# HKUST-Aerial-Robotics/DenseSurfelMapping

Measured on AMD Instinct MI355X. Metric: depth frames fused/sec @ KITTI 1226x370, higher is better.
Workload: dtype f32

## Files before the change

densesurfelmapping_amd/csrc/dsm_api.hip:

```cpp
#include <hip/hip_runtime.h>

#include <cstdarg>
#include <cstdio>
#include <cstdlib>
#include <cstring>
#include <cstdint>
#include <new>
#include <algorithm>
#include <atomic>
#include <condition_variable>
#include <functional>
#include <mutex>
#include <string>
#include <thread>
#include <chrono>
#include <unordered_map>
#include <vector>

#include "dsm_components.h"
#include "dsm_device.h"
#include "dsm_frame_copy.h"
#include "dsm_frame_format.h"
#include "dsm_frame_rings.h"
#include "dsm_ranges.h"
// ... 1033 lines not shown
    CREATE_TRY(dev_alloc(h, &h->d_params, (size_t)kParamRing));
    c.params = h->d_params;
    h->ev_slot.assign((size_t)c.n_slots, nullptr);
    h->slot_used.assign((size_t)c.n_slots, 0);
    CREATE_TRY(hipEventCreateWithFlags(&h->ev_fence, hipEventDisableTiming));
    CREATE_TRY(dev_alloc(h, &h->d_stage_img, (size_t)w * hh));
    CREATE_TRY(dev_alloc(h, &h->d_stage_depth, (size_t)w * hh));
    int np = cfg->pipeline_depth > 0 ? cfg->pipeline_depth : 4;
    if (np != 1 && np != 2 && np != 4 && np != 8 && np != 12 && np != 16 && np != 24 && np != 32) { fail(h, DSM_E_INVALID, "pipeline_depth must be 1, 2, 4, 8, 12, 16, 24 or 32"); return bail(DSM_E_INVALID); }
    if ((cfg->flags & DSM_FLAG_WAVE_STAMPS) && !kWaveStamps) {
        fail(h, DSM_E_INVALID, "DSM_FLAG_WAVE_STAMPS: this library was built without phase stamps (-DDSM_WAVE_STAMPS=1: tools/wave_stamps.py builds such a copy)");
        return bail(DSM_E_INVALID);
    }
    h->n_pipe = np;
    if (np > 1) {
        CREATE_TRY(hipEventCreateWithFlags(&h->ev_params, hipEventDisableTiming));
        CREATE_TRY(hipStreamCreateWithFlags(&h->copy_stream, hipStreamNonBlocking));
    }
    for (int p = 0; p < np; p++) {
        dsm_handle::Pipe &pp = h->pipe[p];
        pp.ctx = c;
        DeviceCtx &q = pp.ctx;
        q.cursor_mul = np; q.cursor_add = p;
        if (np > 1) {
            if (np >= 4 && p < kBatchStreams - ((np == 12 || np == 24) ? 1 : 0)) pp.stream = batch_stream_at(h->device, p);
            if (pp.stream) pp.own_stream = false;
            else CREATE_TRY(hipStreamCreateWithFlags(&pp.stream, hipStreamNonBlocking));
            CREATE_TRY(hipEventCreateWithFlags(&pp.ev_sp, hipEventDisableTiming));
            CREATE_TRY(hipEventCreateWithFlags(&pp.ev_map, hipEventDisableTiming));
        }
        CREATE_TRY(dev_alloc(h, &q.label, (size_t)c.slot_elems));
        CREATE_TRY(dev_alloc(h, &q.cand, (size_t)c.slot_elems));
        CREATE_TRY(dev_alloc(h, &q.worklist, (size_t)c.slot_elems));
        CREATE_TRY(dev_alloc(h, &q.core, (size_t)c.n_seed));
        CREATE_TRY(dev_alloc(h, &q.inv_depth, (size_t)c.n_seed));
        CREATE_TRY(dev_alloc(h, &q.core_stage, (size_t)c.n_seed));
        CREATE_TRY(dev_alloc(h, &q.stable_stage, (size_t)c.n_seed));
        CREATE_TRY(dev_alloc(h, &q.tmin, (size_t)c.n_seed));
        CREATE_TRY(dev_alloc(h, &q.first_empty, (size_t)kSweeps * kWorkers));
        CREATE_TRY(dev_alloc(h, &q.gn_hdr, (size_t)c.n_seed));
        CREATE_TRY(dev_alloc(h, &q.normals, (size_t)c.slot_elems * 3));
        CREATE_TRY(dev_alloc(h, &q.plane, (size_t)c.n_seed));
        CREATE_TRY(dev_alloc(h, &q.seeds, (size_t)c.n_seed));
        CREATE_TRY(dev_alloc(h, &q.spawn_rec, (size_t)c.n_seed));
        CREATE_TRY(dev_alloc(h, &q.spawn_ok, (size_t)c.n_seed));
        CREATE_TRY(dev_alloc(h, &q.fused_flag, (size_t)c.n_seed));
        CREATE_TRY(dev_alloc(h, &q.seed_weight, (size_t)c.n_seed));
        CREATE_TRY(dev_alloc(h, &q.spawn_idx, (size_t)c.n_seed));
        int32_t *ps = nullptr;
        CREATE_TRY(dev_alloc(h, &ps, 64));
        q.work_count = ps + 0; q.cursor = ps + 8; q.fit_big_count = ps + 24; q.rest_count = ps + 32;
        q.fit_small_cap = kFitSmallCap;
        CREATE_TRY(dev_alloc(h, &q.cur, 1));
        CREATE_TRY(dev_alloc(h, &q.rest_list, (size_t)((c.n_seed + 63) / 64) * kRestListCap * 64));
        CREATE_TRY(dev_alloc(h, &q.inl_mask, (size_t)((c.n_seed + 63) / 64) * (2 * kCell) * 64));
        if ((cfg->flags & DSM_FLAG_WAVE_STAMPS) && kWaveStamps) CREATE_TRY(dev_alloc(h, &q.stamps, (size_t)5 * c.n_seed * 8));
        q.params = h->d_params;
        if (np > 1) CREATE_TRY(hipEventRecord(pp.ev_map, h->stream));
    }
    h->hc = h->pipe[0].ctx;
    if (np >= 4) {
        CREATE_TRY(dev_alloc(h, &h->d_pipe_ctxs, (size_t)np));
        DeviceCtx tmp[kMaxPipes];
        for (int p = 0; p < np; p++) tmp[p] = h->pipe[p].ctx;
        CREATE_TRY(hipMemcpyAsync(h->d_pipe_ctxs, tmp, sizeof(DeviceCtx) * (size_t)np, hipMemcpyHostToDevice, h->stream));
        CREATE_TRY(hipStreamSynchronize(h->stream));
    }
    CREATE_TRY(hipHostMalloc((void **)&h->h_params, sizeof(FrameParams) * kParamRing, hipHostMallocDefault));
    CREATE_TRY(hipHostMalloc((void **)&h->h_scalars, 512, hipHostMallocDefault));
    memset(h->h_scalars, 0, 512);
    for (int i = 0; i <= kNumStages + 1; i++) CREATE_TRY(hipEventCreate(&h->ev[i]));
    h->have_events = true;
    CREATE_TRY(hipStreamSynchronize(h->stream));
#undef CREATE_TRY
    (void)rc;
    {
        std::lock_guard<std::mutex> lk(g_live_mu);
        h->generation = g_next_generation++;
        g_live[h] = h->generation;
    }
    *out = h;
    return DSM_OK;
}

void dsm_destroy(dsm_handle *h) {
    if (!h) return;
    {
        std::lock_guard<std::mutex> lk(g_live_mu);
        g_live.erase(h);
    }
    (void)hipSetDevice(h->device);
    if (h->stream && h->batch_order_ev) (void)hipStreamWaitEvent(h->stream, h->batch_order_ev, 0);
    if (h->stream) (void)hipStreamSynchronize(h->stream);
    retire_graphs(h);
    for (int i = 0; i < 4; i++) {
        if (h->g_group[i]) (void)hipGraphExecDestroy(h->g_group[i]);
        if (h->g_group_map[i]) (void)hipGraphExecDestroy(h->g_group_map[i]);
        if (h->g_group_map_large[i]) (void)hipGraphExecDestroy(h->g_group_map_large[i]);
    }
    for (int p = 0; p < kMaxPipes; p++) {
        dsm_handle::Pipe &pp = h->pipe[p];
        if (pp.stream) (void)hipStreamSynchronize(pp.stream);
        if (pp.g_sp) (void)hipGraphExecDestroy(pp.g_sp);
        if (pp.g_sp_main) (void)hipGraphExecDestroy(pp.g_sp_main);
        for (int i = 0; i < 2; i++) {
            if (pp.g_map[i]) (void)hipGraphExecDestroy(pp.g_map[i]);
// ... 1634 lines not shown
    HIP_TRY(h, hipMemcpy(core4, h->hc.core, S * 16, hipMemcpyDeviceToHost));
    HIP_TRY(h, hipMemcpy(stable, h->hc.tmin, S * 4, hipMemcpyDeviceToHost));
    for (size_t i = 0; i < S; i++) stable[i] = stable[i] == kIntMax ? 1 : 0;
    return DSM_OK;
}

int dsm_debug_set_seed_state(dsm_handle *h, const float *core4, const int32_t *stable) {
    if (!h || !core4 || !stable) return DSM_E_INVALID;
    int rc = bind_device(h);
    if (rc) return rc;
    HIP_TRY(h, hipStreamSynchronize(h->stream));
    const size_t S = (size_t)h->hc.n_seed;
    std::vector<double> inv(S);
    std::vector<int32_t> t(S);
    for (size_t i = 0; i < S; i++) {
        inv[i] = 1.0 / (double)core4[4 * i + 3];
        t[i] = stable[i] ? kIntMax : -1;
    }
    HIP_TRY(h, hipMemcpy(h->hc.core, core4, S * 16, hipMemcpyHostToDevice));
    HIP_TRY(h, hipMemcpy(h->hc.inv_depth, inv.data(), S * 8, hipMemcpyHostToDevice));
    HIP_TRY(h, hipMemcpy(h->hc.tmin, t.data(), S * 4, hipMemcpyHostToDevice));
    return DSM_OK;
}

int dsm_debug_set_fit_small_cap(dsm_handle *h, int32_t cap) {
    if (!h) return DSM_E_INVALID;
    if (cap < 0 || cap > kFitSmallCap) return fail(h, DSM_E_INVALID, "fit_small_cap %d out of range [0, %d]", cap, kFitSmallCap);
    if (h->frames_submitted != 0) return fail(h, DSM_E_STATE, "dsm_debug_set_fit_small_cap: the handle has already fused frames");
    if (h->batches_joined != 0) return fail(h, DSM_E_STATE, "dsm_debug_set_fit_small_cap: the handle has already joined a batch (which holds a copy of its context)");
    int rc = bind_device(h);
    if (rc) return rc;
    for (int p = 0; p < h->n_pipe; p++) h->pipe[p].ctx.fit_small_cap = cap;
    h->hc.fit_small_cap = cap;
    if (h->d_pipe_ctxs) {
        DeviceCtx tmp[kMaxPipes];
        for (int p = 0; p < h->n_pipe; p++) tmp[p] = h->pipe[p].ctx;
        HIP_TRY(h, hipMemcpy(h->d_pipe_ctxs, tmp, sizeof(DeviceCtx) * (size_t)h->n_pipe, hipMemcpyHostToDevice));
    }
    return DSM_OK;
}

int dsm_debug_dropin_stats(dsm_handle *h, int64_t *out ) {
    if (!h || !out) return DSM_E_INVALID;
    out[0] = h->dropin_calls; out[1] = h->dropin_delta_calls; out[2] = h->dropin_delta_groups; out[3] = h->dropin_last_groups;
    for (int i = 0; i < 4; i++) out[4 + i] = (int64_t)h->dropin_us[i];
    return DSM_OK;
}

int dsm_debug_tier_counts(dsm_handle *h, int32_t *out ) {
    if (!h || !out) return DSM_E_INVALID;
    int rc = bind_device(h);
    if (rc) return rc;
    HIP_TRY(h, hipStreamSynchronize(h->stream));
    HIP_TRY(h, hipMemcpy(out, h->hc.rest_count, 6 * sizeof(int32_t), hipMemcpyDeviceToHost));
    HIP_TRY(h, hipMemcpy(out + 6, h->hc.fit_big_count, sizeof(int32_t), hipMemcpyDeviceToHost));
    out[7] = 0;
    return DSM_OK;
}

int dsm_debug_get_frame(dsm_handle *h, int slot, uint8_t *image, float *depth) {
    if (!h) return DSM_E_INVALID;
    if (slot < 0 || slot >= h->hc.n_slots) return fail(h, DSM_E_INVALID, "frame slot %d out of range [0,%d)", slot, h->hc.n_slots);
    int rc = bind_device(h);
    if (rc) return rc;
    {
        const ReadSlots reads(h, slot, slot + 1);
        if ((rc = wait_uploads(h, h->stream, kSerialBit))) return rc;
    }
    HIP_TRY(h, hipStreamSynchronize(h->stream));
    const size_t w = (size_t)h->hc.w, hh = (size_t)h->hc.h, pitch = (size_t)h->hc.pitch;
    if (image) HIP_TRY(h, hipMemcpy2D(image, w, (const uint8_t *)h->hc.img_base + (int64_t)slot * h->hc.slot_elems, pitch, w, hh, hipMemcpyDeviceToHost));
    if (depth) HIP_TRY(h, hipMemcpy2D(depth, w * 4, (const float *)h->hc.depth_base + (int64_t)slot * h->hc.slot_elems, pitch * 4, w * 4, hh, hipMemcpyDeviceToHost));
    return DSM_OK;
}

int dsm_debug_frame_planes(dsm_handle *h, int slot, int write, uint8_t *image, float *depth) {
    if (!h) return DSM_E_INVALID;
    if (slot < 0 || slot >= h->hc.n_slots) return fail(h, DSM_E_INVALID, "frame slot %d out of range [0,%d)", slot, h->hc.n_slots);
    int rc = bind_device(h);
    if (rc) return rc;
    {
        const ReadSlots reads(h, slot, slot + 1);
        if ((rc = wait_uploads(h, h->stream, kSerialBit))) return rc;
    }
    HIP_TRY(h, hipStreamSynchronize(h->stream));
    const size_t plane = (size_t)h->hc.pitch * (size_t)h->hc.h;
    uint8_t *di = (uint8_t *)h->hc.img_base + (int64_t)slot * h->hc.slot_elems;
    float *dd = (float *)h->hc.depth_base + (int64_t)slot * h->hc.slot_elems;
    if (image) HIP_TRY(h, write ? hipMemcpy(di, image, plane, hipMemcpyHostToDevice) : hipMemcpy(image, di, plane, hipMemcpyDeviceToHost));
    if (depth) HIP_TRY(h, write ? hipMemcpy(dd, depth, plane * 4, hipMemcpyHostToDevice) : hipMemcpy(depth, dd, plane * 4, hipMemcpyDeviceToHost));
    return DSM_OK;
}

int dsm_debug_wave_stamps(dsm_handle *h, int64_t *out ) {
    if (!h || !out) return DSM_E_INVALID;
    if (!kWaveStamps) return fail(h, DSM_E_STATE, "this library was built without phase stamps (-DDSM_WAVE_STAMPS=1: tools/wave_stamps.py builds such a copy)");
    if (!h->hc.stamps) return fail(h, DSM_E_STATE, "handle was created without DSM_FLAG_WAVE_STAMPS");
    int rc = bind_device(h);
    if (rc) return rc;
    HIP_TRY(h, hipStreamSynchronize(h->stream));
    HIP_TRY(h, hipMemcpy(out, h->hc.stamps, (size_t)5 * h->hc.n_seed * 8 * sizeof(int64_t), hipMemcpyDeviceToHost));
    return DSM_OK;
}

}

namespace {
// ... 330 lines not shown
```

densesurfelmapping_amd/csrc/dsm_k_superpixel.h:

```cpp
#pragma once
#include "dsm_k_common.h"

namespace dsm {

constexpr int kInitLanes = 16, kInitSeedsPerBlock = 256 / kInitLanes;
template <bool BATCH> __global__ __launch_bounds__(256) void k_init_seeds(const DeviceCtx ctx, const DeviceCtx *__restrict__ batch) {
    const BlockOf blk = block_of<BATCH>();
    DeviceCtx batch_ctx;
    if (BATCH) batch_ctx = load_ctx(batch + blk.z);
    const DeviceCtx *__restrict__ c = BATCH ? &batch_ctx : &ctx;
    const int tid = threadIdx.x, lane = lane_id();
    const int r = tid & (kInitLanes - 1);
    const int s = blk.x * kInitSeedsPerBlock + tid / kInitLanes;
    if (blk.x == 0 && tid < kSweeps * kWorkers) c->first_empty[tid] = kIntMax;
    if (blk.x == 0 && tid == 0) c->work_count[0] = c->fit_big_count[0] = 0;
    if (blk.x == 0 && tid < 2 * kSweeps) c->rest_count[tid] = 0;
    const FrameParams &fp = c->params[(unsigned)(c->cursor[0] * c->cursor_mul + c->cursor_add) % (unsigned)c->n_params];
    const uint8_t *img = c->img_base + (int64_t)fp.slot * c->slot_elems;
    const float *dep = c->depth_base + (int64_t)fp.slot * c->slot_elems;
    if (blk.x == 0 && tid < 64) {
        FrameCur *wc = c->cur;
        const int t = tid;
        if (t < 16) wc->p.pose[t] = fp.pose[t];
        else if (t < 32) wc->p.inv[t - 16] = fp.inv[t - 16];
        else if (t == 32) { wc->p.ref_idx = fp.ref_idx; wc->p.slot = fp.slot; }
        else if (t == 33) wc->img = img;
        else if (t == 34) wc->dep = dep;
    }
    const int w = c->w, h = c->h, pitch = c->pitch;
    const bool live = s < c->n_seed;
    const int sc = live ? s : 0;
    const int gx = sc % c->gw, gy = sc / c->gw;
    int ix = gx * kCell + kCell / 2, iy = gy * kCell + kCell / 2;
    if (ix > w - 1) ix = w - 1;
    if (iy > h - 1) iy = h - 1;
    const int wx0 = gx * kCell + kCell / 2 - kCell, wy0 = gy * kCell + kCell / 2 - kCell;
    const int x_lo = wx0 < 0 ? 0 : wx0, x_hi = wx0 + 2 * kCell > w - 1 ? w - 1 : wx0 + 2 * kCell;
    const int y_lo = wy0 < 0 ? 0 : wy0, y_hi = wy0 + 2 * kCell > h - 1 ? h - 1 : wy0 + 2 * kCell;
    const int y = wy0 + r;
    const bool row_in = y >= y_lo && y < y_hi;
    float md = dep[iy * pitch + ix];
    const float mi = (float)img[iy * pitch + ix];
    float4 v[4];
#pragma unroll
    for (int q = 0; q < 4; q++) {
        const int x = wx0 + 4 * q;
        v[q] = (row_in && x >= 0) ? *reinterpret_cast<const float4 *>(dep + y * pitch + x) : make_float4(0, 0, 0, 0);
    }
    bool hit = false;
    float first = 0.0f;
#pragma unroll
    for (int q = 3; q >= 0; q--) {
        const float e[4] = {v[q].x, v[q].y, v[q].z, v[q].w};
#pragma unroll
        for (int t = 3; t >= 0; t--) {
            const int x = wx0 + 4 * q + t;
            if (row_in && x >= x_lo && x < x_hi && e[t] > flt_below(0.01)) { hit = true; first = e[t]; }
        }
    }
    const unsigned long long m = __ballot(hit);
    const unsigned rows = (unsigned)(m >> (lane & ~(kInitLanes - 1))) & 0xffffu;
    const int src = (lane & ~(kInitLanes - 1)) + (rows ? __ffs((int)rows) - 1 : 0);
    const float scanned = __shfl(first, src);
    if (md < flt_above(0.01) && rows) md = scanned;
    if (!live || r != 0) return;
    c->core[s] = make_float4((float)ix, (float)iy, mi, md);
    c->inv_depth[s] = 1.0 / (double)md;
    c->tmin[s] = -1;
}

template <bool BATCH> __global__ __launch_bounds__(256) void k_init_seeds_lanes(const DeviceCtx ctx, const DeviceCtx *__restrict__ batch) {
    const BlockOf blk = block_of<BATCH>();
    DeviceCtx batch_ctx;
    if (BATCH) batch_ctx = load_ctx(batch + blk.z);
    const DeviceCtx *__restrict__ c = BATCH ? &batch_ctx : &ctx;
    const int tid = threadIdx.x;
    const int s = blk.x * 256 + tid;
    if (blk.x == 0 && tid < kSweeps * kWorkers) c->first_empty[tid] = kIntMax;
    if (blk.x == 0 && tid == 0) c->work_count[0] = c->fit_big_count[0] = 0;
    if (blk.x == 0 && tid < 2 * kSweeps) c->rest_count[tid] = 0;
    const FrameParams &fp = c->params[(unsigned)(c->cursor[0] * c->cursor_mul + c->cursor_add) % (unsigned)c->n_params];
    const uint8_t *img = c->img_base + (int64_t)fp.slot * c->slot_elems;
    const float *dep = c->depth_base + (int64_t)fp.slot * c->slot_elems;
    if (blk.x == 0 && tid < 64) {
        FrameCur *wc = c->cur;
        const int t = tid;
        if (t < 16) wc->p.pose[t] = fp.pose[t];
        else if (t < 32) wc->p.inv[t - 16] = fp.inv[t - 16];
        else if (t == 32) { wc->p.ref_idx = fp.ref_idx; wc->p.slot = fp.slot; }
        else if (t == 33) wc->img = img;
        else if (t == 34) wc->dep = dep;
    }
    const int w = c->w, h = c->h, pitch = c->pitch;
    const bool live = s < c->n_seed;
    const int sc = live ? s : 0;
    int gx, gy;
    seed_cell(c, sc, gx, gy);
    int ix = gx * kCell + kCell / 2, iy = gy * kCell + kCell / 2;
    if (ix > w - 1) ix = w - 1;
    if (iy > h - 1) iy = h - 1;
    float md = dep[iy * pitch + ix];
    const float mi = (float)img[iy * pitch + ix];
    const bool need = live && md < flt_above(0.01);
    if (__ballot(need) != 0) {
        const int wx0 = gx * kCell + kCell / 2 - kCell, wy0 = gy * kCell + kCell / 2 - kCell;
        const int x_lo = wx0 < 0 ? 0 : wx0, x_hi = wx0 + 2 * kCell > w - 1 ? w - 1 : wx0 + 2 * kCell;
        const int y_lo = wy0 < 0 ? 0 : wy0, y_hi = wy0 + 2 * kCell > h - 1 ? h - 1 : wy0 + 2 * kCell;
        bool pending = need;
#pragma unroll 1
        for (int r0 = 0; r0 < 2 * kCell && __ballot(pending) != 0; r0 += 2) {
            float4 v[2][4];
            bool row_in[2];
#pragma unroll
            for (int k = 0; k < 2; k++) {
                const int y = wy0 + r0 + k;
                row_in[k] = pending && y >= y_lo && y < y_hi;
#pragma unroll
                for (int q = 0; q < 4; q++) {
                    const int x = wx0 + 4 * q;
                    v[k][q] = (row_in[k] && x >= 0) ? *reinterpret_cast<const float4 *>(dep + y * pitch + x) : make_float4(0, 0, 0, 0);
                }
            }
#pragma unroll
            for (int k = 0; k < 2; k++) {
                bool hit = false;
                float first = 0.0f;
#pragma unroll
                for (int q = 3; q >= 0; q--) {
                    const float e[4] = {v[k][q].x, v[k][q].y, v[k][q].z, v[k][q].w};
#pragma unroll
                    for (int t = 3; t >= 0; t--) {
                        const int x = wx0 + 4 * q + t;
                        if (row_in[k] && x >= x_lo && x < x_hi && e[t] > flt_below(0.01)) { hit = true; first = e[t]; }
// ... 329 lines not shown
        pimg[k] = x_in && y >= 0 && y < h;
        const int pk = pimg[k] ? key0 + k * row4 : 0;
        const unsigned o4 = (unsigned)pk << 2;
        lab[k] = (int)ld_off(lbl, (unsigned)pk << 1);
        pd[k] = ld_off(dep, o4);
        pi[k] = (int)ld_off(img, (unsigned)pk);
    }
#pragma unroll
    for (int k = 0; k < 4; k++) {
        const int idx = k * 64 + lane;
        const int y = y0 + 4 * k;
        const bool mem = pimg[k] && x < w - 1 && y < h - 1 && lab[k] == s;
        const float d = mem ? pd[k] : 0.0f;
        if (mem) {
            cnt += 1; sdx += idx & (kWin - 1); sdy += idx >> 4; si += pi[k];
        }
        const bool dv = mem && d > flt_below(0.1);
        const unsigned long long m = __ballot(dv);
        if (dv) dl[nd + rank_below(m)] = d;
        nd += __popcll(m);
    }
    update_seed_finish(c, sweep, s, lane, wx0, wy0, old, dl, lt, cnt, sdx, sdy, si, nd);
}

template <typename Fetch> __device__ __forceinline__ float huber_pass_lanes(Fetch fetch, int lim, float md, double hr) {
    const float hr_above = flt_above(hr);
    const unsigned hr_lo = (unsigned)__double_as_longlong(hr), hr_hi = (unsigned)(__double_as_longlong(hr) >> 32);
    float a = 0.0f;
    int n_tail = 0;
    float d8[8];
#pragma unroll
    for (int q = 0; q < 8; q++) d8[q] = fetch(q);
    for (int i = 0; __ballot(i < lim) != 0; i += 8) {
        float n8[8];
#pragma unroll
        for (int q = 0; q < 8; q++) n8[q] = fetch(i + 8 + q);
#pragma unroll
        for (int q = 0; q < 8; q++) {
            const float r = i + q < lim ? md - d8[q] : 0.0f;
            const bool core = fabsf(r) < hr_above;
            const float a_core = a + 2 * r;
            const double step = __longlong_as_double((long long)(((unsigned long long)(r > 0 ? hr_hi : hr_hi ^ 0x80000000u) << 32) | hr_lo));
            const float a_tail = (float)((double)a + step);
            a = core ? a_core : a_tail;
            n_tail += core ? 0 : 1;
        }
#pragma unroll
        for (int q = 0; q < 8; q++) d8[q] = n8[q];
    }
    const float b = (float)(2 * (lim - n_tail));
    return huber_newton_step(a, b);
}

constexpr int kRestRegs = 128;
__device__ __forceinline__ float huber_pass_regs(const float (&v)[kRestRegs], int lim, float md, double hr) {
    const float hr_above = flt_above(hr);
    const unsigned hr_lo = (unsigned)__double_as_longlong(hr), hr_hi = (unsigned)(__double_as_longlong(hr) >> 32);
    float a = 0.0f;
    int n_tail = 0;
#pragma unroll
    for (int i = 0; i < kRestRegs; i += 8) {
        if (__ballot(i < lim) == 0) break;
#pragma unroll
        for (int q = 0; q < 8; q++) {
            const float r = i + q < lim ? md - v[i + q] : 0.0f;
            const bool core = fabsf(r) < hr_above;
            const float a_core = a + 2 * r;
            const double step = __longlong_as_double((long long)(((unsigned long long)(r > 0 ? hr_hi : hr_hi ^ 0x80000000u) << 32) | hr_lo));
            const float a_tail = (float)((double)a + step);
            a = core ? a_core : a_tail;
            n_tail += core ? 0 : 1;
        }
    }
    const float b = (float)(2 * (lim - n_tail));
    return huber_newton_step(a, b);
}

constexpr int kLaneCap = kRestListCap;
enum { kQueueRest = 0, kQueueWave = 1 };
__device__ __forceinline__ int32_t *queue_wave(const DeviceCtx *c) { return c->worklist + 4 * c->n_seed; }
__device__ __forceinline__ int32_t *fit_order(const DeviceCtx *c) { return c->worklist + 4 * c->n_seed; }

struct LaneRow {
    LabelQuad lab[4];
    float4 dp[4];
    unsigned im[4];
};

template <bool BATCH> __global__ __launch_bounds__(64) void k_update_seeds(const DeviceCtx ctx, const DeviceCtx *__restrict__ batch, int sweep) {
    constexpr int CAP = kLaneCap - 3;
    const BlockOf blk = block_of<BATCH>();
    DeviceCtx batch_ctx;
    if (BATCH) batch_ctx = load_ctx(batch + blk.z);
    const DeviceCtx *__restrict__ c = BATCH ? &batch_ctx : &ctx;
    __shared__ __attribute__((aligned(16))) float s_list[(CAP + 4) * 64];
    const int lane = lane_id();
    const int S = c->n_seed;
    const FrameParams &fp = frame_params(c);
    const uint8_t *img = frame_image(c, fp);
    const float *dep = frame_depth(c, fp);
    const label_t *lbl = c->label;
    const int w = c->w, h = c->h, pitch = c->pitch;
    const int s = (((S + 63) >> 6) - 1 - blk.x) * 64 + lane;
    const bool live = s < S;
    const int sc = live ? s : S - 1;
    int gx, gy;
    seed_cell(c, sc, gx, gy);
    const int wx0 = gx * kCell + kCell / 2 - kCell, wy0 = gy * kCell + kCell / 2 - kCell;
    const int t_self = c->tmin[sc];
    const float4 old = c->core[sc];
    const bool stats = live && t_self != kIntMax;
    const unsigned s_match = stats ? (unsigned)s : (unsigned)kNoSeed;
    int qx[4];
#pragma unroll
    for (int q = 0; q < 4; q++) {
        const int x = wx0 + 4 * q;
        qx[q] = x < 0 ? 0 : (x > pitch - 4 ? pitch - 4 : x);
    }
    unsigned s_col[kWin];
#pragma unroll
    for (int j = 0; j < kWin; j++) s_col[j] = (unsigned)(wx0 + j) < (unsigned)(w - 1) ? s_match : (unsigned)kNoSeed;

    auto load_row = [&](int r) {
        LaneRow R;
        int y = wy0 + r;
        y = y < 0 ? 0 : (y > h - 1 ? h - 1 : y);
        const unsigned row = (unsigned)__mul24(y, pitch);
#pragma unroll
        for (int q = 0; q < 4; q++) {
            const unsigned o = row + (unsigned)qx[q], o4 = o << 2;
            R.lab[q] = label_quad(lbl, o);
            R.dp[q] = ld_vec<float4>(dep, o4);
            R.im[q] = ld_vec<unsigned>(img, o);
        }
        return R;
    };

    int acc_ci = 0;
    int colcnt[kWin];
#pragma unroll
    for (int j = 0; j < kWin; j++) colcnt[j] = 0;
    int acc_y = 0, cnt_prev = 0;
    const unsigned lane4 = (unsigned)lane << 2, tail_cap = ((unsigned)CAP << 8) + lane4;
    unsigned tail = lane4;
    float sum = 0.0f;

    auto process_row = [&](const LaneRow &A, int r) {
        const int y = wy0 + r;
        if ((unsigned)y < (unsigned)(h - 1)) {
#pragma unroll
            for (int j = 0; j < kWin; j++) {
                const bool mem = comp(A.lab[j >> 2], j & 3) == s_col[j];
                const int pi = (int)((A.im[j >> 2] >> (8 * (j & 3))) & 0xffu);
                acc_ci += mem ? pi | 0x10000 : 0;
                colcnt[j] += mem ? 1 : 0;
                const float d = comp(A.dp[j >> 2], j & 3);
                const float dm = mem ? d : 0.0f;
                const bool dv = dm > flt_below(0.1);
                if ((j & 3) == 0) tail = tail < tail_cap ? tail : tail_cap;
                *reinterpret_cast<float *>(reinterpret_cast<char *>(s_list) + tail) = d;
                tail += dv ? 256u : 0u;
                sum += dv ? dm : 0.0f;
                if ((j & 3) == 3) {
                    asm volatile("" : "+v"(acc_ci), "+v"(sum), "+v"(tail), "+v"(colcnt[j - 3]), "+v"(colcnt[j - 2]), "+v"(colcnt[j - 1]), "+v"(colcnt[j]));
                    __builtin_amdgcn_sched_barrier(0);
                }
            }
        }
        const int cnt_now = acc_ci >> 16;
        acc_y += r * (cnt_now - cnt_prev);
        cnt_prev = cnt_now;
    };

    LaneRow B0 = load_row(0), B1 = load_row(1), B2 = load_row(2), B3;
#pragma unroll 1
    for (int r = 0; r < kWin; r += 4) {
        B3 = load_row(r + 3);
        __builtin_amdgcn_sched_barrier(0);
        process_row(B0, r);
        if (r + 4 < kWin) B0 = load_row(r + 4);
        __builtin_amdgcn_sched_barrier(0);
        process_row(B1, r + 1);
        if (r + 4 < kWin) B1 = load_row(r + 5);
        __builtin_amdgcn_sched_barrier(0);
        process_row(B2, r + 2);
        if (r + 4 < kWin) B2 = load_row(r + 6);
        __builtin_amdgcn_sched_barrier(0);
        process_row(B3, r + 3);
    }

    const int cnt = acc_ci >> 16, si = acc_ci & 0xffff;
    const int nd = (int)((tail - lane4) >> 8);
    const bool empty = stats && cnt == 0;
    if (empty) atomicMin(&c->first_empty[sweep * kWorkers + chunk_of(S, s)], s);
    const bool settled = sum == __builtin_inff();
    const bool over = stats && nd >= CAP && !settled;
    const bool fin = stats && cnt > 0 && !over;
    int acc_x = 0;
#pragma unroll
    for (int j = 1; j < kWin; j++) acc_x += j * colcnt[j];
    const int sx = acc_x + cnt * wx0, sy = acc_y + cnt * wy0;
    const float fn = (float)cnt;
    const float mi = (float)si / fn, mx = (float)sx / fn, my = (float)sy / fn;
    const float moved = fabsf(old.z - mi) + fabsf(old.x - mx) + fabsf(old.y - my);
    const int stable = moved < flt_above(0.2) ? 1 : 0;
    float md = 0.0f;
    bool run = fin && nd > 0;
    if (run) md = sum / (float)nd;
    run = run && !settled;
    const double hr = c->huber;
    wave_lds_sync();
    if (__ballot(run) != 0) {
        const float delta = huber_pass_lanes([&](int i) { return s_list[(i < CAP ? i : CAP) * 64 + lane]; }, run ? nd : 0, md, hr);
        if (run) md = md + delta;
        if (fabsf(delta) < flt_above(0.01)) run = false;
    }
    const unsigned long long rm = __ballot(run), om = __ballot(over);
    if (rm | om) {
        int base_r = 0, base_o = 0;
        if (lane == 0) {
            if (rm) base_r = atomicAdd(&c->rest_count[2 * sweep + kQueueRest], __popcll(rm));
            if (om) base_o = atomicAdd(&c->rest_count[2 * sweep + kQueueWave], __popcll(om));
        }
        base_r = __builtin_amdgcn_readfirstlane(base_r);
        base_o = __builtin_amdgcn_readfirstlane(base_o);
        if (over) queue_wave(c)[base_o + rank_below(om)] = s;
        const int q = base_r + rank_below(rm);
        if (run) reinterpret_cast<int4 *>(c->worklist)[q] = make_int4(s, nd, __float_as_int(md), 0);
        const unsigned dst0 = (((unsigned)(q >> 6) * kLaneCap) << 8) + ((unsigned)(q & 63) << 2);
        const int lim = run ? nd : 0;
        for (int i = 0; __ballot(i < lim) != 0; i += 4) {
#pragma unroll
            for (int t = 0; t < 4; t++)
                if (i + t < lim) st_off(c->rest_list, dst0 + ((unsigned)(i + t) << 8), s_list[(i + t) * 64 + lane]);
        }
    }
    if (fin) {
        c->core_stage[s] = make_float4(mx, my, mi, md);
        c->stable_stage[s] = stable;
    }
}

constexpr int kRestOverBlocks = 128;
constexpr int kLaneBatch = 8;
template <bool BATCH> __global__ __launch_bounds__(64) void k_update_seeds_rest(const DeviceCtx ctx, const DeviceCtx *__restrict__ batch, int sweep) {
    const BlockOf blk = block_of<BATCH>();
    DeviceCtx batch_ctx;
    if (BATCH) batch_ctx = load_ctx(batch + blk.z);
    const DeviceCtx *__restrict__ c = BATCH ? &batch_ctx : &ctx;
    __shared__ __attribute__((aligned(16))) float s_depth[kWin * kWin], s_term[kWin * kWin];
    const int lane = lane_id();
    const int S = c->n_seed, n_dense = (S + 63) >> 6;
    if (blk.x >= n_dense) {
        const int n_over = c->rest_count[2 * sweep + kQueueWave];
        for (int e = blk.x - n_dense; e < n_over; e += kRestOverBlocks) {
            update_seed_wave(c, sweep, __builtin_amdgcn_readfirstlane(queue_wave(c)[e]), s_depth, s_term);
            wave_lds_sync();
        }
        return;
    }
    const int n = c->rest_count[2 * sweep + kQueueRest];
    if (blk.x * 64 >= n) return;
    const int q = blk.x * 64 + lane;
    const bool live = q < n;
    const int4 ent = reinterpret_cast<const int4 *>(c->worklist)[live ? q : blk.x * 64];
    const int s = ent.x, nd = ent.y;
    float md = __int_as_float(ent.z);
    const double hr = c->huber;
    const unsigned src0 = (((unsigned)blk.x * kLaneCap) << 8) + ((unsigned)lane << 2);
    const int n_max = __builtin_amdgcn_readfirstlane(wave_max_int(live ? nd : 0));
    static_assert(kRestRegs >= kLaneCap, "list registers");
    float v[kRestRegs];
#pragma unroll
    for (int b = 0; b < kRestRegs; b += 16) {
        if (b < n_max) {
#pragma unroll
            for (int q = 0; q < 16; q++) v[b + q] = ld_off(c->rest_list, src0 + ((unsigned)(b + q < n_max ? b + q : n_max - 1) << 8));
        } else {
#pragma unroll
            for (int q = 0; q < 16; q++) v[b + q] = 0.0f;
        }
    }
    bool run = live;
#pragma unroll 1
    for (int it = 1; it < 5; it++) {
        if (__ballot(run) == 0) break;
        const float delta = huber_pass_regs(v, run ? nd : 0, md, hr);
        if (run) md = md + delta;
        if (fabsf(delta) < flt_above(0.01)) run = false;
    }
    if (live) c->core_stage[s].w = md;
}

template <bool BATCH> __global__ __launch_bounds__(256) void k_update_seeds_wave(const DeviceCtx ctx, const DeviceCtx *__restrict__ batch, int sweep) {
    const BlockOf blk = block_of<BATCH>();
    DeviceCtx batch_ctx;
    if (BATCH) batch_ctx = load_ctx(batch + blk.z);
    const DeviceCtx *__restrict__ c = BATCH ? &batch_ctx : &ctx;
    __shared__ __attribute__((aligned(16))) float s_depth[4][kWin * kWin];
    __shared__ __attribute__((aligned(16))) float s_term[4][kWin * kWin];
    const int wv = threadIdx.x >> 6;
    const int s = __builtin_amdgcn_readfirstlane(seed_of_block(blk.x, wv, c->gw, c->gh));
    if (s < 0) return;
    update_seed_wave(c, sweep, s, s_depth[wv], s_term[wv]);
}

template <bool BATCH> __global__ __launch_bounds__(256) void k_commit_seeds(const DeviceCtx ctx, const DeviceCtx *__restrict__ batch, int sweep) {
    const BlockOf blk = block_of<BATCH>();
    DeviceCtx batch_ctx;
    if (BATCH) batch_ctx = load_ctx(batch + blk.z);
    const DeviceCtx *__restrict__ c = BATCH ? &batch_ctx : &ctx;
    const int s = blk.x * 256 + threadIdx.x;
    if (s == 0) c->work_count[0] = 0;
    if (s >= c->n_seed) return;
    if (c->tmin[s] == kIntMax) return;
    int t = -1;
    if (s < c->first_empty[sweep * kWorkers + chunk_of(c->n_seed, s)]) {
        const float4 v = c->core_stage[s];
        c->core[s] = v;
        c->inv_depth[s] = 1.0 / (double)v.w;
        if (c->stable_stage[s]) t = kIntMax;
    }
    c->tmin[s] = t;
}


}
```

densesurfelmapping_amd/csrc/dsm_math.h:

```cpp
#pragma once
#include <math.h>
#include <stdint.h>

#if defined(__HIPCC__) || defined(__HIP__)
#define DSM_HD __host__ __device__ __forceinline__
#else
#define DSM_HD static inline
#endif

namespace dsm {

constexpr int kCell = 8;
constexpr int kSweeps = 3;
constexpr int kWorkers = 10;
constexpr double kAngleCos = 0.1;

struct Intrinsics {
    float fx, fy, cx, cy;
};

DSM_HD constexpr float flt_below(double c) {
    const float f = (float)c;
    return (double)f <= c ? f : __builtin_bit_cast(float, __builtin_bit_cast(uint32_t, f) - 1u);
}
// ... 176 lines not shown
        const f32x2 ddyq = f2_sub(q.sy4[j], yq);
        const f32x2 dist16 = f2_fma(ddyq, ddyq, edge ? q.ax16_edge[j] : q.ax16[j]);
        const f32x2 t = f2_mul(f2_sub(q.si[j], pi), tenth);
        const f32x2 c_no = f2_fma(t, t, dist16);
        dd20[j] = f2_fma(q.s20[j], mm, p20m);
        c[j] = f2_fma(dd20[j], dd20[j], c_no);
    }
    const float ck[4] = {c[0].x, c[0].y, c[1].x, c[1].y};
    const float ad_max = fmaxf(fmaxf(fabsf(dd20[0].x), fabsf(dd20[0].y)), fmaxf(fabsf(dd20[1].x), fabsf(dd20[1].y)));
    uint32_t key[4];
    for (int k = 0; k < 4; k++) key[k] = (__builtin_bit_cast(uint32_t, ck[k]) & ~3u) | (uint32_t)k;
    const uint32_t lo01 = key[0] < key[1] ? key[0] : key[1], hi01 = key[0] < key[1] ? key[1] : key[0];
    const uint32_t lo23 = key[2] < key[3] ? key[2] : key[3], hi23 = key[2] < key[3] ? key[3] : key[2];
    const uint32_t first = lo01 < lo23 ? lo01 : lo23;
    const uint32_t mid_a = lo01 < lo23 ? lo23 : lo01, mid_b = hi01 < hi23 ? hi01 : hi23;
    const uint32_t second = mid_a < mid_b ? mid_a : mid_b;
    const float c1 = __builtin_bit_cast(float, first), c2 = fminf(__builtin_bit_cast(float, second), 2e6f);
    const float err = fast_cost_err(c2, fast_cost_slack(ad_max, q.df));
    if (trace) { trace->err = err; trace->all_depth = all_depth; }
    FastPick r;
    r.seed = q.base + (int)(first & 1u) * gw + (int)((first >> 1) & 1u);
    r.sure = c1 + err < c2 - err && c1 + err < 1e6f;
    return r;
}
template <typename LoadSeedF>
DSM_HD FastPick pick_seed_fast(int x, int y, float pix_i, float pix_d, int gw, int gh, LoadSeedF load, FastPickTrace *trace = nullptr) {
    return pick_seed_fast(pick_col(x, y, gw, gh, load), y, pix_i, pix_d, gw, trace);
}

DSM_HD float huber_newton_step(float a, float b) { return (-a) / (b + 10.0f); }

DSM_HD bool mean_depth_is_settled(float md) { return md == __builtin_inff(); }

DSM_HD float huber_mean_depth(const float *list, int n, float sum, double huber) {
    const float hr_above = flt_above(huber);
    float md = sum / (float)n;
    if (mean_depth_is_settled(md)) return md;
    for (int it = 0; it < 5; it++) {
        float a = 0, b = 0;
        for (int k = 0; k < n; k++) {
            float r = md - list[k];
            if (fabsf(r) < hr_above) {
                a += 2 * r;
                b += 2;
            } else {
                a = (float)((double)a + (r > 0 ? huber : -1 * huber));
            }
        }
        float delta = huber_newton_step(a, b);
        md = md + delta;
        if (fabsf(delta) < flt_above(0.01)) break;
    }
    return md;
}

struct WindowPixel {
    bool member, has_depth, inlier;
};
DSM_HD WindowPixel window_pixel(bool row_in, bool col_in, bool label_is_seed, float d, float mean_depth, float hr_above) {
    WindowPixel p;
    p.member = row_in && col_in && label_is_seed;
    p.has_depth = p.member && d > flt_below(0.05);
    p.inlier = p.has_depth && fabsf(mean_depth - d) < hr_above;
    return p;
}

DSM_HD void back_project(const Intrinsics &k, float u, float v, float d, float &x, float &y, float &z) {
    x = (u - k.cx) / k.fx * d;
    y = (v - k.cy) / k.fy * d;
    z = d;
}

DSM_HD float ray_coeff(int u, float c, float f) { return ((float)u - c) / f; }

DSM_HD bool pixel_normal_rays(float rx0, float rx1, float ry0, float ry1, float d, float d_right, float d_down, float &nx, float &ny,
                              float &nz) {
    constexpr float kMin = flt_above(0.1);
    if (d < kMin || d_right < kMin || d_down < kMin) return false;
    const float px = rx0 * d, py = ry0 * d, pz = d;
    float rx = rx1 * d_right, ry = ry0 * d_right, rz = d_right;
    float dx = rx0 * d_down, dy = ry1 * d_down, dz = d_down;
    rx = rx - px; ry = ry - py; rz = rz - pz;
    dx = dx - px; dy = dy - py; dz = dz - pz;
    float ax = ry * dz - rz * dy, ay = rz * dx - rx * dz, az = rx * dy - ry * dx;
    float len = sqrtf(ax * ax + ay * ay + az * az);
    ax /= len; ay /= len; az /= len;
    float va = (ax * px + ay * py + az * pz) / sqrtf(px * px + py * py + pz * pz);
    if (fabsf(va) < flt_above(kAngleCos)) return false;
    nx = ax; ny = ay; nz = az;
    return true;
}

DSM_HD bool pixel_normal(const Intrinsics &k, int x, int y, float d, float d_right, float d_down, float &nx,
                         float &ny, float &nz) {
    constexpr float kMin = flt_above(0.1);
    if (d < kMin || d_right < kMin || d_down < kMin) return false;
    float px, py, pz, rx, ry, rz, dx, dy, dz;
    back_project(k, (float)x, (float)y, d, px, py, pz);
    back_project(k, (float)(x + 1), (float)y, d_right, rx, ry, rz);
    back_project(k, (float)x, (float)(y + 1), d_down, dx, dy, dz);
    rx = rx - px; ry = ry - py; rz = rz - pz;
    dx = dx - px; dy = dy - py; dz = dz - pz;
    float ax = ry * dz - rz * dy, ay = rz * dx - rx * dz, az = rx * dy - ry * dx;
    float len = sqrtf(ax * ax + ay * ay + az * az);
    ax /= len; ay /= len; az /= len;
    float va = (ax * px + ay * py + az * pz) / sqrtf(px * px + py * py + pz * pz);
// ... 487 lines not shown
```

Baseline: 46770.

## Use udot4 for window stats and a core-only first Huber pass

The per-row window accumulation now packs membership flags into bytes and uses udot4 to accumulate count, intensity sum and column-weighted sum. This replaces the per-column counters and the packed acc_ci word, cutting register pressure and ALU work. The first Huber pass in the wave path now assumes every element is inside the core, so b is simply 2n and the double-precision branch is skipped. If any lane finds an outlier, that seed is marked for restart and the full iteration runs in the rest kernel, which now tracks the iteration count per seed. A new first-pass counter tap is added to rest_count, which adds an atomic and extends the debug readout.

After: 47270, median of 6. 1.1% higher.

```diff
diff --git a/densesurfelmapping_amd/csrc/dsm_api.hip b/densesurfelmapping_amd/csrc/dsm_api.hip
--- a/densesurfelmapping_amd/csrc/dsm_api.hip
+++ b/densesurfelmapping_amd/csrc/dsm_api.hip
@@ -1109,6 +1109,7 @@
         q.work_count = ps + 0; q.cursor = ps + 8; q.fit_big_count = ps + 24; q.rest_count = ps + 32;
         q.fit_small_cap = kFitSmallCap;
         CREATE_TRY(dev_alloc(h, &q.cur, 1));
+        static_assert(kCell * kCell >= 5, "worklist holds the pass queue (4 words a seed) and the wave queue (1)");
         CREATE_TRY(dev_alloc(h, &q.rest_list, (size_t)((c.n_seed + 63) / 64) * kRestListCap * 64));
         CREATE_TRY(dev_alloc(h, &q.inl_mask, (size_t)((c.n_seed + 63) / 64) * (2 * kCell) * 64));
         if ((cfg->flags & DSM_FLAG_WAVE_STAMPS) && kWaveStamps) CREATE_TRY(dev_alloc(h, &q.stamps, (size_t)5 * c.n_seed * 8));
@@ -2849,7 +2850,12 @@
     int rc = bind_device(h);
     if (rc) return rc;
     HIP_TRY(h, hipStreamSynchronize(h->stream));
-    HIP_TRY(h, hipMemcpy(out, h->hc.rest_count, 6 * sizeof(int32_t), hipMemcpyDeviceToHost));
+    int32_t rc9[3 * kSweeps];
+    HIP_TRY(h, hipMemcpy(rc9, h->hc.rest_count, sizeof(rc9), hipMemcpyDeviceToHost));
+    for (int s = 0; s < kSweeps; s++) {
+        out[2 * s + 0] = rc9[2 * kSweeps + s];
+        out[2 * s + 1] = rc9[2 * s + 1];
+    }
     HIP_TRY(h, hipMemcpy(out + 6, h->hc.fit_big_count, sizeof(int32_t), hipMemcpyDeviceToHost));
     out[7] = 0;
     return DSM_OK;
diff --git a/densesurfelmapping_amd/csrc/dsm_k_superpixel.h b/densesurfelmapping_amd/csrc/dsm_k_superpixel.h
--- a/densesurfelmapping_amd/csrc/dsm_k_superpixel.h
+++ b/densesurfelmapping_amd/csrc/dsm_k_superpixel.h
@@ -14,7 +14,7 @@
     const int s = blk.x * kInitSeedsPerBlock + tid / kInitLanes;
     if (blk.x == 0 && tid < kSweeps * kWorkers) c->first_empty[tid] = kIntMax;
     if (blk.x == 0 && tid == 0) c->work_count[0] = c->fit_big_count[0] = 0;
-    if (blk.x == 0 && tid < 2 * kSweeps) c->rest_count[tid] = 0;
+    if (blk.x == 0 && tid < 3 * kSweeps) c->rest_count[tid] = 0;
     const FrameParams &fp = c->params[(unsigned)(c->cursor[0] * c->cursor_mul + c->cursor_add) % (unsigned)c->n_params];
     const uint8_t *img = c->img_base + (int64_t)fp.slot * c->slot_elems;
     const float *dep = c->depth_base + (int64_t)fp.slot * c->slot_elems;
@@ -78,7 +78,7 @@
     const int s = blk.x * 256 + tid;
     if (blk.x == 0 && tid < kSweeps * kWorkers) c->first_empty[tid] = kIntMax;
     if (blk.x == 0 && tid == 0) c->work_count[0] = c->fit_big_count[0] = 0;
-    if (blk.x == 0 && tid < 2 * kSweeps) c->rest_count[tid] = 0;
+    if (blk.x == 0 && tid < 3 * kSweeps) c->rest_count[tid] = 0;
     const FrameParams &fp = c->params[(unsigned)(c->cursor[0] * c->cursor_mul + c->cursor_add) % (unsigned)c->n_params];
     const uint8_t *img = c->img_base + (int64_t)fp.slot * c->slot_elems;
     const float *dep = c->depth_base + (int64_t)fp.slot * c->slot_elems;
@@ -514,6 +514,26 @@
     return huber_newton_step(a, b);
 }
 
+template <typename Fetch> __device__ __forceinline__ float huber_core_pass_lanes(Fetch fetch, int lim, float md, float hr_above, bool &tail) {
+    float a = 0.0f;
+    unsigned long long outside = 0;
+    float d0[8], d1[8];
+#pragma unroll
+    for (int q = 0; q < 8; q++) d0[q] = fetch(0, q);
+    for (int i = 0; __ballot(i < lim) != 0; i += 16) {
+#pragma unroll
+        for (int q = 0; q < 8; q++) d1[q] = fetch(i + 8, q);
+#pragma unroll
+        for (int q = 0; q < 8; q++) outside |= __ballot(huber_core_only_element(a, i + q < lim, md, d0[q], hr_above));
+#pragma unroll
+        for (int q = 0; q < 8; q++) d0[q] = fetch(i + 16, q);
+#pragma unroll
+        for (int q = 0; q < 8; q++) outside |= __ballot(huber_core_only_element(a, i + 8 + q < lim, md, d1[q], hr_above));
+    }
+    tail = ((outside >> lane_id()) & 1ull) != 0;
+    return a;
+}
+
 constexpr int kRestRegs = 128;
 __device__ __forceinline__ float huber_pass_regs(const float (&v)[kRestRegs], int lim, float md, double hr) {
     const float hr_above = flt_above(hr);
@@ -540,6 +560,7 @@
 
 constexpr int kLaneCap = kRestListCap;
 enum { kQueueRest = 0, kQueueWave = 1 };
+constexpr int kTapFirstPass = 2 * kSweeps;
 __device__ __forceinline__ int32_t *queue_wave(const DeviceCtx *c) { return c->worklist + 4 * c->n_seed; }
 __device__ __forceinline__ int32_t *fit_order(const DeviceCtx *c) { return c->worklist + 4 * c->n_seed; }
 
@@ -598,10 +619,7 @@
         return R;
     };
 
-    int acc_ci = 0;
-    int colcnt[kWin];
-#pragma unroll
-    for (int j = 0; j < kWin; j++) colcnt[j] = 0;
+    unsigned acc_n = 0, acc_i = 0, acc_x = 0;
     int acc_y = 0, cnt_prev = 0;
     const unsigned lane4 = (unsigned)lane << 2, tail_cap = ((unsigned)CAP << 8) + lane4;
     unsigned tail = lane4;
@@ -610,12 +628,11 @@
     auto process_row = [&](const LaneRow &A, int r) {
         const int y = wy0 + r;
         if ((unsigned)y < (unsigned)(h - 1)) {
+            unsigned flags = 0;
 #pragma unroll
             for (int j = 0; j < kWin; j++) {
                 const bool mem = comp(A.lab[j >> 2], j & 3) == s_col[j];
-                const int pi = (int)((A.im[j >> 2] >> (8 * (j & 3))) & 0xffu);
-                acc_ci += mem ? pi | 0x10000 : 0;
-                colcnt[j] += mem ? 1 : 0;
+                flags |= mem ? 1u << (8 * (j & 3)) : 0u;
                 const float d = comp(A.dp[j >> 2], j & 3);
                 const float dm = mem ? d : 0.0f;
                 const bool dv = dm > flt_below(0.1);
@@ -624,12 +641,17 @@
                 tail += dv ? 256u : 0u;
                 sum += dv ? dm : 0.0f;
                 if ((j & 3) == 3) {
-                    asm volatile("" : "+v"(acc_ci), "+v"(sum), "+v"(tail), "+v"(colcnt[j - 3]), "+v"(colcnt[j - 2]), "+v"(colcnt[j - 1]), "+v"(colcnt[j]));
+                    const unsigned cols = 0x03020100u + 0x04040404u * (unsigned)(j >> 2);
+                    acc_n = __builtin_amdgcn_udot4(flags, 0x01010101u, acc_n, false);
+                    acc_i = __builtin_amdgcn_udot4(flags, A.im[j >> 2], acc_i, false);
+                    acc_x = __builtin_amdgcn_udot4(flags, cols, acc_x, false);
+                    flags = 0;
+                    asm volatile("" : "+v"(acc_n), "+v"(acc_i), "+v"(acc_x), "+v"(sum), "+v"(tail));
                     __builtin_amdgcn_sched_barrier(0);
                 }
             }
         }
-        const int cnt_now = acc_ci >> 16;
+        const int cnt_now = (int)acc_n;
         acc_y += r * (cnt_now - cnt_prev);
         cnt_prev = cnt_now;
     };
@@ -651,17 +673,14 @@
         process_row(B3, r + 3);
     }
 
-    const int cnt = acc_ci >> 16, si = acc_ci & 0xffff;
+    const int cnt = (int)acc_n, si = (int)acc_i;
     const int nd = (int)((tail - lane4) >> 8);
     const bool empty = stats && cnt == 0;
     if (empty) atomicMin(&c->first_empty[sweep * kWorkers + chunk_of(S, s)], s);
     const bool settled = sum == __builtin_inff();
     const bool over = stats && nd >= CAP && !settled;
     const bool fin = stats && cnt > 0 && !over;
-    int acc_x = 0;
-#pragma unroll
-    for (int j = 1; j < kWin; j++) acc_x += j * colcnt[j];
-    const int sx = acc_x + cnt * wx0, sy = acc_y + cnt * wy0;
+    const int sx = (int)acc_x + cnt * wx0, sy = acc_y + cnt * wy0;
     const float fn = (float)cnt;
     const float mi = (float)si / fn, mx = (float)sx / fn, my = (float)sy / fn;
     const float moved = fabsf(old.z - mi) + fabsf(old.x - mx) + fabsf(old.y - my);
@@ -672,10 +691,17 @@
     run = run && !settled;
     const double hr = c->huber;
     wave_lds_sync();
+    bool restart = false;
     if (__ballot(run) != 0) {
-        const float delta = huber_pass_lanes([&](int i) { return s_list[(i < CAP ? i : CAP) * 64 + lane]; }, run ? nd : 0, md, hr);
-        if (run) md = md + delta;
-        if (fabsf(delta) < flt_above(0.01)) run = false;
+        bool met_tail;
+        const float a = huber_core_pass_lanes([&](int i0, int q) { return s_list[((i0 < CAP - 4 ? i0 : CAP - 4) + q) * 64 + lane]; }, run ? nd : 0, md, flt_above(hr), met_tail);
+        const float delta = huber_newton_step(a, (float)(2 * nd));
+        restart = run && met_tail;
+        const bool stepped = run && !met_tail && !(fabsf(delta) < flt_above(0.01));
+        if (run && !met_tail) md = md + delta;
+        const unsigned long long sm = __ballot(stepped);
+        if (sm != 0 && lane == 0) atomicAdd(&c->rest_count[kTapFirstPass + sweep], __popcll(sm));
+        run = stepped || restart;
     }
     const unsigned long long rm = __ballot(run), om = __ballot(over);
     if (rm | om) {
@@ -688,7 +714,7 @@
         base_o = __builtin_amdgcn_readfirstlane(base_o);
         if (over) queue_wave(c)[base_o + rank_below(om)] = s;
         const int q = base_r + rank_below(rm);
-        if (run) reinterpret_cast<int4 *>(c->worklist)[q] = make_int4(s, nd, __float_as_int(md), 0);
+        if (run) reinterpret_cast<int4 *>(c->worklist)[q] = make_int4(s, nd, __float_as_int(md), restart ? 0 : 1);
         const unsigned dst0 = (((unsigned)(q >> 6) * kLaneCap) << 8) + ((unsigned)(q & 63) << 2);
         const int lim = run ? nd : 0;
         for (int i = 0; __ballot(i < lim) != 0; i += 4) {
@@ -743,13 +769,21 @@
             for (int q = 0; q < 16; q++) v[b + q] = 0.0f;
         }
     }
+    int it = ent.w;
+    const bool restarted = live && it == 0;
     bool run = live;
 #pragma unroll 1
-    for (int it = 1; it < 5; it++) {
+    for (int trip = 0; trip < 5; trip++) {
         if (__ballot(run) == 0) break;
         const float delta = huber_pass_regs(v, run ? nd : 0, md, hr);
         if (run) md = md + delta;
-        if (fabsf(delta) < flt_above(0.01)) run = false;
+        const bool small = fabsf(delta) < flt_above(0.01);
+        if (trip == 0) {
+            const unsigned long long sm = __ballot(restarted && !small);
+            if (sm != 0 && lane == 0) atomicAdd(&c->rest_count[kTapFirstPass + sweep], __popcll(sm));
+        }
+        it += 1;
+        if (small || it >= 5) run = false;
     }
     if (live) c->core_stage[s].w = md;
 }
diff --git a/densesurfelmapping_amd/csrc/dsm_math.h b/densesurfelmapping_amd/csrc/dsm_math.h
--- a/densesurfelmapping_amd/csrc/dsm_math.h
+++ b/densesurfelmapping_amd/csrc/dsm_math.h
@@ -252,6 +252,49 @@
         if (fabsf(delta) < flt_above(0.01)) break;
     }
     return md;
+}
+
+DSM_HD bool huber_core_only_element(float &a, bool in_list, float md, float d, float hr_above) {
+    const float r = in_list ? md - d : 0.0f;
+    const bool core = fabsf(r) < hr_above;
+    a = a + 2 * r;
+    return !core;
+}
+
+DSM_HD float huber_mean_depth_from(const float *list, int n, float md, double huber, int start) {
+    const float hr_above = flt_above(huber);
+    for (int it = start; it < 5; it++) {
+        float a = 0, b = 0;
+        for (int k = 0; k < n; k++) {
+            float r = md - list[k];
+            if (fabsf(r) < hr_above) {
+                a += 2 * r;
+                b += 2;
+            } else {
+                a = (float)((double)a + (r > 0 ? huber : -1 * huber));
+            }
+        }
+        float delta = huber_newton_step(a, b);
+        md = md + delta;
+        if (fabsf(delta) < flt_above(0.01)) break;
+    }
+    return md;
+}
+
+enum HuberRoute { kHuberSettled = 0, kHuberDoneFirst = 1, kHuberMorePasses = 2, kHuberRestart = 3 };
+DSM_HD float huber_mean_depth_routed(const float *list, int n, float sum, double huber, int *route) {
+    const float hr_above = flt_above(huber);
+    float md = sum / (float)n;
+    if (mean_depth_is_settled(md)) { *route = kHuberSettled; return md; }
+    float a = 0.0f;
+    bool tail = false;
+    for (int k = 0; k < n; k++) tail = huber_core_only_element(a, true, md, list[k], hr_above) || tail;
+    if (tail) { *route = kHuberRestart; return huber_mean_depth_from(list, n, md, huber, 0); }
+    const float delta = huber_newton_step(a, (float)(2 * n));
+    md = md + delta;
+    if (fabsf(delta) < flt_above(0.01)) { *route = kHuberDoneFirst; return md; }
+    *route = kHuberMorePasses;
+    return huber_mean_depth_from(list, n, md, huber, 1);
 }
 
 struct WindowPixel {
```
